# heyblackC/DFMIR

Hardware: AMD Instinct MI355X
Metric: train-step image-pairs/sec (fwd+bwd): 2D 256x256 bs=16 and 3D 160^3 bs=1 (higher is better)
Workload: dtype f32 (fp16x2-split MFMA, fp32 accumulate)

## Files before the change

### dfmir_amd/csrc/conv3x3s.hip

```cpp
#include "split_f16.h"

#ifndef PP_COMPUTE_PRIO
#define PP_COMPUTE_PRIO 1
#endif
#ifndef CS_COMPUTE_PRIO
#define CS_COMPUTE_PRIO 1
#endif
#ifndef CS_STORE_PRIO
#define CS_STORE_PRIO 0
#endif
typedef __bf16 bf16x8 __attribute__((ext_vector_type(8)));
typedef __bf16 bf16x2 __attribute__((ext_vector_type(2)));
typedef _Float16 f16x2 __attribute__((ext_vector_type(2)));
typedef float f32x2 __attribute__((ext_vector_type(2)));

__device__ __forceinline__ unsigned pk_bf16(float a, float b) {
  const f32x2 v = {a, b};
  return __builtin_bit_cast(unsigned, __builtin_convertvector(v, bf16x2));
}

template <int NSP>
__device__ __forceinline__ void split_pair(float x0, float x1, unsigned (&p)[NSP]) {
  if constexpr (NSP == 3) {
    p[0] = pk_bf16(x0, x1);
// ... 581 lines not shown
  const int th = g->Cout > 64 ? 8 : 16;
  const int tx = (g->Wo + CS_TW - 1) / CS_TW, ty = (g->Ho + th - 1) / th;
  const double fill = (double)g->Ho * g->Wo / ((double)tx * CS_TW * ty * th);
  if (!((long long)g->N * tx * ty < (1LL << 31) && fill >= 0.85)) return false;
  *th_out = th; *tx_out = tx; *ty_out = ty;
  return true;
}
static bool split_fwd_geom_ok(const DfConvGeom* g) {
  if (!(g->KD == 1 && g->KH == 3 && g->KW == 3 && g->Di == 1 && g->Do == 1 && g->stride == 1 && g->dil == 1))
    return false;
  if (g->Cout <= 32 || g->Cin < 16 || g->ph != g->pw || g->pd != 0) return false;
  const int p = g->ph;
  if (!(p == 1 || (p == 2 && g->pad_mode == 0))) return false;
  if (g->Ho != g->Hi + 2 * p - 2 || g->Wo != g->Wi + 2 * p - 2) return false;
  const long long HWo = (long long)g->Ho * g->Wo;
  if (HWo >= (1LL << 30) || (long long)g->Hi * g->Wi >= (1LL << 30)) return false;
  if ((long long)((g->Cin + 7) / 8) * 27 * g->Cout * 16 >= (1LL << 31)) return false;
  if (worst_npos(g->Wo, (int)HWo, 128) > 399) return false;
  return true;
}
int df_conv3x3_split_res_ok(const DfConvGeom* g) {
  int th, tx, ty;
  return (df_split_mode() == 2 && split_fwd_geom_ok(g) && cs_plan(g, &th, &tx, &ty)) ? 1 : 0;
}
struct CsLaunch {
  ConvCsP kc;
  dim3 grid;
  int form;
};
static bool cs_setup(const DfConvGeom* g, const float* res, const float* ring, int ring_rl, const float* y, CsLaunch* L) {
  int th = 0, tlx = 0, tly = 0;
  if (!cs_plan(g, &th, &tlx, &tly)) return false;
  ConvCsP kc{g->N, g->Cin, g->Cout, g->Hi, g->Wi, g->Ho, g->Wo, g->ph, g->pad_mode, g->act, g->slope, tlx, tly, res,
             ring, ring_rl, 0, 0, 0};
  kc.vec4 = (g->Wo % 4 == 0 && ((uintptr_t)y & 15) == 0 && ((uintptr_t)res & 15) == 0) ? 1 : 0;
  static DfOptInt dephase_o{"DFMIR_CS_DEPHASE", 0};
  const long long nb = (long long)g->N * tlx * tly;
  if (nb * ((g->Cout + 127) / 128) >= 512) kc.dephase = dephase_o.get();
  static DfOptInt xcd_o{"DFMIR_CS_XCD_PAIR", 2};
  const int xcd_pair = xcd_o.get();
  if (g->Cout > 64) {
    dim3 grid((unsigned)nb, (unsigned)((g->Cout + 127) / 128));
    if (xcd_pair && grid.y <= 2 && (nb & 7) == 0) {
      kc.xcd_pair = xcd_pair == 1 ? (grid.y == 2 ? 1 : 0) : (int)grid.y + 1;
      if (kc.xcd_pair) grid = dim3((unsigned)(grid.y * nb), 1u);
    }
    L->grid = grid;
    L->form = 1;
  } else {
    if (xcd_pair >= 2 && (nb & 7) == 0) kc.xcd_pair = 2;
    L->grid = dim3((unsigned)nb, 1u);
    L->form = 2;
  }
  L->kc = kc;
  return true;
}
bool df_conv3x3_split_fwd_try(const DfConvGeom* g, const float* x, const float* x_amax, int x_n, const float* w_packed,
                              const float* bias, const float* res, const float* ring, int ring_rl, float* y,
                              hipStream_t st, int* rc) {
  const int mode = df_split_mode();
  if (mode == 0 || (mode == 2 && !(x_amax && x_n > 0))) return false;
  if (!split_fwd_geom_ok(g)) return false;
  const int p = g->ph;
  const long long HWo = (long long)g->Ho * g->Wo;
  Conv3P k{g->N, g->Cin, g->Cout, g->Hi, g->Wi, g->Ho, g->Wo, p, g->pad_mode, g->act, g->slope, 0};
  const u32x4* ws = reinterpret_cast<const u32x4*>(split_section(w_packed, g->Cin, g->Cout));
  const SplitScale sc{x_amax, x_n, split_trailer(w_packed, g->Cin, g->Cout, mode)};
  CsLaunch cl;
  if (mode == 2 && cs_setup(g, res, ring, ring_rl, y, &cl)) {
    const ConvCsP& kc = cl.kc;
    if (cl.form == 1) {
#ifdef DFMIR_BUILD_W1
      static DfOptFlag w1_o{"DFMIR_CONV_W1"};
      if (w1_o.get() && kc.vec4 && g->act != 2 && (g->Cin % 16) == 0 && (g->Ho % 16) == 0 && (g->Wo % 32) == 0) {
        ConvCsP kw = kc;
        kw.tiles_y = g->Ho / 16;
        const long long nbw = (long long)g->N * kw.tiles_x * kw.tiles_y;
        const unsigned gyw = (unsigned)((g->Cout + 127) / 128);
        kw.xcd_pair = 0;
        dim3 gw((unsigned)nbw, gyw);
        if ((nbw & 7) == 0 && gyw <= 2) { kw.xcd_pair = (int)gyw + 1; gw = dim3((unsigned)(gyw * nbw), 1u); }
        conv3x3_split_w1_k<0><<<gw, 256, 0, st>>>(x, ws, bias, y, kw, sc);
      } else
#endif
      conv3x3_split_cs_k<64, 8><<<cl.grid, 512, 0, st>>>(x, ws, bias, y, kc, sc);
    } else {
      conv3x3_split_cs_k<32, 16><<<cl.grid, 512, 0, st>>>(x, ws, bias, y, kc, sc);
    }
    hipError_t e = hipGetLastError();
    *rc = (e == hipSuccess) ? 0 : df_set_error((int)e, __FILE__, __LINE__);
    return true;
  }
  if (res || ring) { *rc = df_set_error((int)hipErrorInvalidValue, __FILE__, __LINE__); return true; }
  k.tiles_per_img = (int)((HWo + 255) / 256);
  const bool big = g->Cout > 64;
  dim3 grid((unsigned)(g->N * k.tiles_per_img), big ? (unsigned)((g->Cout + 127) / 128) : 1u);
  if (mode == 2) {
    if (big) conv3x3_split_pp_k<2, 400, 128><<<grid, 512, 0, st>>>(x, ws, bias, y, k, sc);
    else conv3x3_split_pp_k<2, 400, 64><<<grid, 512, 0, st>>>(x, ws, bias, y, k, sc);
  } else {
    if (big) conv3x3_split_pp_k<3, 400, 128><<<grid, 512, 0, st>>>(x, ws, bias, y, k, sc);
    else conv3x3_split_pp_k<3, 400, 64><<<grid, 512, 0, st>>>(x, ws, bias, y, k, sc);
  }
  hipError_t e = hipGetLastError();
  *rc = (e == hipSuccess) ? 0 : df_set_error((int)e, __FILE__, __LINE__);
  return true;
}

struct WS3P {
  int N, Cin, Cout, H, W, pad_mode;
  int runs_per_row, runs_per_img, runs_total, runs_per_block;
  const float* x_amax;
  const float* dy_amax;
  int x_n, dy_n;
  float* db;
  const float* dy_pmax;
  int swap;
  float* dbx;
  const float* fx;
};

template <int NSP, int BC>
__global__ __launch_bounds__(512, 1) void conv3x3_wgrad_split_k(const float* __restrict__ x,
                                                                const float* __restrict__ dy,
                                                                float* __restrict__ dwt, WS3P k) {
  using P = Prod<NSP>;
  constexpr int CT = 64, NWC = BC / 32, KS = 4 / NWC, NSTEP = 18 / KS;
  constexpr int XSLAB = 2 * CT;
  __shared__ __attribute__((aligned(16))) u32x4 Xc[NSP * 3 * 4 * XSLAB];
  __shared__ __attribute__((aligned(16))) u32x4 Dy[NSP * 2 * 2 * BC];
  __shared__ float bsum[BC];

  const int tid = threadIdx.x, lane = tid & 63, wid = tid >> 6;
  const bool want_db = k.db != nullptr && blockIdx.y == 0;
  if (tid < BC) bsum[tid] = 0.f;
  float bacc = 0.f;
  const int wc = wid % NWC, wi = (wid / NWC) & 1, kh = wid / (2 * NWC);
  const int l31 = lane & 31, lhi = lane >> 5;
  const int HW = k.H * k.W;
  const int ci0 = blockIdx.y * CT, co0 = blockIdx.z * BC;
  const int run_beg = blockIdx.x * k.runs_per_block;
  int run_end = run_beg + k.runs_per_block;
  if (run_end > k.runs_total) run_end = k.runs_total;

  float xscale = 1.f, dscale = 1.f, oscale = 1.f, oscale2 = 1.f;
  if (NSP == 2) {
    __shared__ float red[17];
    const int ex = scale_exp(reduce_absmax(k.x_amax, k.x_n, red));
    __syncthreads();
    const int ed = scale_exp(reduce_absmax(k.dy_amax, k.dy_n, red));
    xscale = pow2f(ex); dscale = pow2f(ed); oscale = pow2f(-ex); oscale2 = pow2f(-ed);
  }

  const int xc = tid & 63, xu = (tid >> 6) & 1, xr = tid >> 7;
  const int dc = tid % BC, du = (tid / BC) & 1, dk = (tid / (2 * BC)) & 1;
  const bool dload = tid < 4 * BC;
  const unsigned hw4 = (unsigned)HW * 4u;
  constexpr unsigned OOB = 0x80000000u;

  f32x16 acc[9];
#pragma unroll
  for (int t = 0; t < 9; ++t)
#pragma unroll
    for (int r = 0; r < 16; ++r) acc[t][r] = 0.f;

  u32x4 rxa, rxb, rda, rdb;
  unsigned rxl, rxr;

#define WS_GLOAD(run_)                                                                           \
  {                                                                                              \
    const int n_ = (run_) / k.runs_per_img;                                                      \
    const int q_ = (run_) - n_ * k.runs_per_img;                                                 \
    const int yp_ = q_ / k.runs_per_row, xs_ = q_ - yp_ * k.runs_per_row;                        \
    const int y0_ = 2 * yp_, x0_ = 16 * xs_ + 8 * xu;                                            \
    const __amdgpu_buffer_rsrc_t bx_ = __builtin_amdgcn_make_buffer_rsrc(                        \
        const_cast<float*>(x + (long long)n_ * k.Cin * HW), 0, (unsigned)(k.Cin * HW) * 4u, 0x00020000); \
    const __amdgpu_buffer_rsrc_t bd_ = __builtin_amdgcn_make_buffer_rsrc(                        \
        const_cast<float*>(dy + (long long)n_ * k.Cout * HW), 0, (unsigned)(k.Cout * HW) * 4u, 0x00020000); \
    const bool cok_ = ci0 + xc < k.Cin;                                                          \
    const unsigned cb_ = (unsigned)(ci0 + xc) * hw4;                                             \
     \
                                             \
    int ry_ = y0_ - 1 + xr;                                                                      \
    bool rok_ = (unsigned)ry_ < (unsigned)k.H;                                                   \
    if (k.pad_mode == 1) { ry_ = ry_ < 0 ? -ry_ : (ry_ >= k.H ? 2 * (k.H - 1) - ry_ : ry_); rok_ = true; } \
    const int rb_ = ry_ * k.W;                                                                   \
    const bool lin_ = x0_ > 0, rin_ = x0_ + 8 < k.W;                                             \
    const int ol_ = rb_ + (lin_ ? x0_ - 1 : 1), or_ = rb_ + (rin_ ? x0_ + 8 : k.W - 2);          \
    const bool lok_ = rok_ && cok_ && (lin_ || k.pad_mode == 1), rrok_ = rok_ && cok_ && (rin_ || k.pad_mode == 1); \
    const unsigned xb_ = (rok_ && cok_) ? cb_ + (unsigned)(rb_ + x0_) * 4u : OOB;                \
    rxa = __builtin_amdgcn_raw_buffer_load_b128(bx_, xb_, 0, 0);                                 \
    rxb = __builtin_amdgcn_raw_buffer_load_b128(bx_, xb_ == OOB ? OOB : xb_ + 16u, 0, 0);        \
    rxl = __builtin_amdgcn_raw_buffer_load_b32(bx_, lok_ ? cb_ + (unsigned)ol_ * 4u : OOB, 0, 0); \
    rxr = __builtin_amdgcn_raw_buffer_load_b32(bx_, rrok_ ? cb_ + (unsigned)or_ * 4u : OOB, 0, 0); \
    const unsigned db_ = (co0 + dc >= k.Cout || !dload) ? OOB                                    \
        : (unsigned)(co0 + dc) * hw4 + (unsigned)((y0_ + dk) * k.W + 16 * xs_ + 8 * du) * 4u;    \
    rda = __builtin_amdgcn_raw_buffer_load_b128(bd_, db_, 0, 0);                                 \
    rdb = __builtin_amdgcn_raw_buffer_load_b128(bd_, db_ == OOB ? OOB : db_ + 16u, 0, 0);        \
  }
#define WS_LSTORE()                                                                              \
  {                                                                                              \
    float r[10];                                                                                 \
    r[0] = __uint_as_float(rxl); r[9] = __uint_as_float(rxr);                                    \
    _Pragma("unroll") for (int e = 0; e < 4; ++e) { r[1 + e] = __uint_as_float(rxa[e]); r[5 + e] = __uint_as_float(rxb[e]); } \
    unsigned pa[5][NSP], pb[4][NSP];                                                             \
    _Pragma("unroll") for (int i = 0; i < 5; ++i) split_pair_s<NSP>(r[2 * i], r[2 * i + 1], xscale, pa[i]); \
    if (NSP == 2) {             \
      _Pragma("unroll") for (int i = 0; i < 4; ++i)                                              \
        _Pragma("unroll") for (int s = 0; s < NSP; ++s) pb[i][s] = __builtin_amdgcn_alignbit(pa[i + 1][s], pa[i][s], 16); \
    } else {                                                                                     \
      _Pragma("unroll") for (int i = 0; i < 4; ++i) split_pair<NSP>(r[2 * i + 1], r[2 * i + 2], pb[i]); \
    }                                                                                            \
    _Pragma("unroll") for (int s = 0; s < NSP; ++s) {                                            \
      u32x4* dst = Xc + ((s * 3 * 4 + xr) * 2 + xu) * CT + xc;                                   \
      dst[0] = u32x4{pa[0][s], pa[1][s], pa[2][s], pa[3][s]};                                    \
      dst[4 * XSLAB] = u32x4{pb[0][s], pb[1][s], pb[2][s], pb[3][s]};                            \
      dst[8 * XSLAB] = u32x4{pa[1][s], pa[2][s], pa[3][s], pa[4][s]};                            \
    }                                                                                            \
    float v[8];                                                                                  \
    _Pragma("unroll") for (int e = 0; e < 4; ++e) { v[e] = __uint_as_float(rda[e]); v[4 + e] = __uint_as_float(rdb[e]); } \
    bacc += ((v[0] + v[1]) + (v[2] + v[3])) + ((v[4] + v[5]) + (v[6] + v[7]));    \
    u32x4 sp[NSP];                                                                               \
    split8_s<NSP>(v, dscale, sp);                                                                \
    if (dload) { _Pragma("unroll") for (int s = 0; s < NSP; ++s) Dy[((s * 2 + dk) * 2 + du) * BC + dc] = sp[s]; } \
  }

  if (run_beg < run_end) {
    WS_GLOAD(run_beg);
    WS_LSTORE();
  }
  __syncthreads();

  const int abase = lhi * CT + wi * 32 + l31 + (KS == 2 ? kh * XSLAB : 0);
  const int bbase = lhi * BC + wc * 32 + l31 + (KS == 2 ? kh * 2 * BC : 0);
  for (int run = run_beg; run < run_end; ++run) {
    const bool more = (run + 1) < run_end;
    if (more) WS_GLOAD(run + 1);
    u32x4 b[NSP], a[2][NSP];
#define WS_LOADA(set_, step_)                                                                    \
  _Pragma("unroll") for (int s = 0; s < NSP; ++s)                                                \
    a[set_][s] = Xc[((s * 3 + ((step_) % 3)) * 4 + (step_) / 9 + ((step_) % 9) / 3) * XSLAB + abase];
    WS_LOADA(0, 0)
#pragma unroll
    for (int step = 0; step < NSTEP; ++step) {
      if (step % 9 == 0) {
#pragma unroll
        for (int s = 0; s < NSP; ++s) b[s] = Dy[(s * 2 + step / 9) * 2 * BC + bbase];
      }
      if (step + 1 < NSTEP) WS_LOADA((step + 1) & 1, step + 1)
#pragma unroll
      for (int q = 0; q < P::N; ++q)
        acc[step % 9] = mma16<NSP>(a[step & 1][P::A[q]], b[P::B[q]], acc[step % 9]);
    }
#undef WS_LOADA
#pragma unroll
    for (int i = 0; i < 2 * NSP; ++i) __builtin_amdgcn_sched_group_barrier(0x100, 1, 0);
#pragma unroll
    for (int step = 0; step < NSTEP; ++step) {
      const int nr = (step + 1 < NSTEP ? NSP : 0) + ((step + 1) % 9 == 0 && step + 1 < NSTEP ? NSP : 0);
#pragma unroll
      for (int i = 0; i < P::N; ++i) {
        __builtin_amdgcn_sched_group_barrier(0x008, 1, 0);
        if (i < nr) __builtin_amdgcn_sched_group_barrier(0x100, 1, 0);
        if (i == P::N - 1) {
#pragma unroll
          for (int e = P::N; e < nr; ++e) __builtin_amdgcn_sched_group_barrier(0x100, 1, 0);
        }
      }
    }
    if (more) {
      __syncthreads();
      WS_LSTORE();
      __syncthreads();
    }
  }
#undef WS_GLOAD
#undef WS_LSTORE

  if (want_db) {
    if (dload) atomicAdd(&bsum[dc], bacc);
    __syncthreads();
    if (tid < BC && co0 + tid < k.Cout) atomicAdd(&k.db[co0 + tid], bsum[tid]);
  }
  const int co = co0 + wc * 32 + l31;
  if (co < k.Cout) {
#pragma unroll
    for (int t = 0; t < 9; ++t) {
#pragma unroll
      for (int r = 0; r < 16; ++r) {
        const int ci = ci0 + wi * 32 + 4 * lhi + (r & 3) + 8 * (r >> 2);
        if (ci < k.Cin)
          df_acc(dwt, ((long long)t * k.Cin + ci) * k.Cout + co, NSP == 2 ? acc[t][r] * oscale * oscale2 : acc[t][r], k.fx);
      }
    }
  }
}

struct RingP {
  int N, K, M, H, W;
  int RL;
  const float* cols;
};
constexpr int RING_KG = 32;

template <int RP>
__global__ __launch_bounds__(512) void conv3x3_reflect_ring_k(const float* __restrict__ dy, const u32x4* __restrict__ ws,
                                                              float* __restrict__ ring, RingP k, SplitScale sc) {
  constexpr int NSP = 2;
  using P = Prod<2>;
  __shared__ __attribute__((aligned(16))) u32x4 Ls[NSP * RING_KG * RP];
  __shared__ float red[17];
  const int tid = threadIdx.x, lane = tid & 63;
  const int wid = __builtin_amdgcn_readfirstlane((int)(threadIdx.x >> 6));
  const int l31 = lane & 31, lhi = lane >> 5;
  const int strip = blockIdx.x & 3, n = blockIdx.x >> 2;
  const int m0 = blockIdx.y * 128;
  const bool rowstrip = strip < 2;
  const int L = rowstrip ? k.W : k.H;
  const int HW = k.H * k.W;
  const float* dyl = dy + (long long)n * k.K * HW +
                     (strip == 0 ? 0 : strip == 1 ? (k.H - 1) * k.W : strip == 2 ? 0 : k.W - 1);
  const int istr = rowstrip ? 1 : k.W;

  const int ex = scale_exp(reduce_absmax(sc.x_amax, sc.x_n, red));
  const int ew = (int)sc.w_trailer[1];
  const float xscale = pow2f(ex), oscale = pow2f(-ex), oscale2 = pow2f(-ew);

  const int kg_n = (k.K + 7) >> 3;
  {
    const int npad = RP - L;
    for (int it = tid; it < NSP * RING_KG * npad; it += 512) {
      const int q = it % npad, g = it / npad;
      Ls[g * RP + (q < 2 ? q : L + q)] = u32x4{0u, 0u, 0u, 0u};
    }
    const int kz = RING_KG - kg_n;
    for (int it = tid; it < NSP * kz * L; it += 512) {
      const int i = it % L, g = it / L, s2 = g / kz, kg = kg_n + g % kz;
      Ls[(s2 * RING_KG + kg) * RP + i + 2] = u32x4{0u, 0u, 0u, 0u};
    }
  }
  for (int it = tid; it < kg_n * L; it += 512) {
    const int i = it % L, kg = it / L;
    float v[8];
#pragma unroll
    for (int e = 0; e < 8; ++e) {
      const int kk = kg * 8 + e;
      if (!rowstrip && k.cols) v[e] = kk < k.K ? k.cols[(((long long)n * k.K + kk) * 2 + (strip - 2)) * k.H + i] : 0.f;
      else v[e] = kk < k.K ? dyl[(long long)kk * HW + (long long)i * istr] : 0.f;
    }
    u32x4 sp[NSP];
    split8_s<NSP>(v, xscale, sp);
#pragma unroll
    for (int s = 0; s < NSP; ++s) Ls[(s * RING_KG + kg) * RP + i + 2] = sp[s];
  }
  __syncthreads();

  const int mb = wid & 3, kh = wid >> 2;
  const int m = m0 + mb * 32 + l31;
  const int nb_n = (L + 2 + 31) >> 5;
  f32x16 acc[3];
#pragma unroll
  for (int b = 0; b < 3; ++b)
#pragma unroll
    for (int r = 0; r < 16; ++r) acc[b][r] = 0.f;
  const int chunks = (k.K + 15) >> 4;
  const int tap0 = strip == 0 ? 6 : strip == 1 ? 0 : strip == 2 ? 2 : 0, tapd = rowstrip ? 1 : 3;
  u32x4 a[3][NSP], an[3][NSP], an2[3][NSP];
#define RING_LOADA(dst_, c_)                                                                     \
  {                                                                                              \
    const int kg_ = 2 * (c_) + lhi;                                                              \
    const bool ok_ = (c_) < chunks && kg_ < kg_n && m < k.M;                                     \
    _Pragma("unroll") for (int j = 0; j < 3; ++j)                                                \
      _Pragma("unroll") for (int s = 0; s < NSP; ++s)                                            \
        dst_[j][s] = ok_ ? ws[((long long)kg_ * NSP * 9 + s * 9 + tap0 + j * tapd) * k.M + m] : u32x4{0u, 0u, 0u, 0u}; \
  }
  RING_LOADA(a, kh)
  RING_LOADA(an, kh + 2)
  for (int c = kh; c < chunks; c += 2) {
    RING_LOADA(an2, c + 4)
    const int kg = 2 * c + lhi;
#pragma unroll
    for (int j = 0; j < 3; ++j) {
#pragma unroll
      for (int b = 0; b < 3; ++b) {
        if (b < nb_n) {
          int pos = b * 32 + l31 + j;
          pos = pos < RP ? pos : RP - 1;
          u32x4 x2[NSP];
#pragma unroll
          for (int s = 0; s < NSP; ++s) x2[s] = Ls[(s * RING_KG + kg) * RP + pos];
#pragma unroll
          for (int q = 0; q < P::N; ++q) acc[b] = mma16<NSP>(a[j][P::A[q]], x2[P::B[q]], acc[b]);
        }
      }
    }
#pragma unroll
    for (int j = 0; j < 3; ++j)
#pragma unroll
      for (int s = 0; s < NSP; ++s) { a[j][s] = an[j][s]; an[j][s] = an2[j][s]; }
  }
#undef RING_LOADA

  __syncthreads();
  float* xch = reinterpret_cast<float*>(Ls);
  if (kh == 1) {
#pragma unroll
    for (int b = 0; b < 3; ++b)
#pragma unroll
      for (int r = 0; r < 16; ++r) xch[((mb * 3 + b) * 16 + r) * 64 + lane] = acc[b][r];
  }
  __syncthreads();
  if (kh == 1) return;
  float* rg = ring + ((long long)(n * 4 + strip) * k.M) * k.RL;
#pragma unroll
  for (int b = 0; b < 3; ++b) {
    if (b >= nb_n) continue;
    const int c = b * 32 + l31;
    if (c > L + 1) continue;
#pragma unroll
    for (int r = 0; r < 16; ++r) {
      const int mm = m0 + mb * 32 + 4 * lhi + (r & 3) + 8 * (r >> 2);
      if (mm < k.M)
        rg[(long long)mm * k.RL + c] = (acc[b][r] + xch[((mb * 3 + b) * 16 + r) * 64 + lane]) * oscale * oscale2;
    }
  }
}

int df_conv3x3_reflect_ring_ok(const DfConvGeom* g) {
  if (df_split_mode() != 2) return 0;
  if (!(g->KD == 1 && g->KH == 3 && g->KW == 3 && g->Di == 1 && g->Do == 1 && g->stride == 1 && g->dil == 1)) return 0;
  if (g->pad_mode != 1 || g->ph != 1 || g->pw != 1 || g->pd != 0) return 0;
  if (g->Ho != g->Hi || g->Wo != g->Wi || g->Hi < 4 || g->Wi < 4 || g->Hi > 94 || g->Wi > 94) return 0;
  if (g->Cout > 8 * RING_KG || g->Cout < 16 || g->Cin <= 32) return 0;
  return 1;
}
int df_conv3x3_reflect_ring_len(const DfConvGeom* g) { return ((g->Hi > g->Wi ? g->Hi : g->Wi) + 2 + 3) & ~3; }
int df_conv3x3_reflect_ring_launch(const DfConvGeom* g, const float* dy, const float* dy_cols, const float* dy_amax,
                                   int dy_n, const float* wd_packed, float* ring, hipStream_t st) {
  const RingP k{g->N, g->Cout, g->Cin, g->Hi, g->Wi, df_conv3x3_reflect_ring_len(g), dy_cols};
  const u32x4* ws = reinterpret_cast<const u32x4*>(split_section(wd_packed, g->Cout, g->Cin));
  const SplitScale sc{dy_amax, dy_n, split_trailer(wd_packed, g->Cout, g->Cin, 2)};
  const dim3 grid((unsigned)(4 * g->N), (unsigned)((g->Cin + 127) / 128));
  if (g->Hi <= 64 && g->Wi <= 64) conv3x3_reflect_ring_k<72><<<grid, 512, 0, st>>>(dy, ws, ring, k, sc);
  else conv3x3_reflect_ring_k<100><<<grid, 512, 0, st>>>(dy, ws, ring, k, sc);
  return (int)hipGetLastError();
}

#ifdef W2_TRACE
__device__ unsigned g_w2_trace[8 * 64 * 8];
extern "C" int dfmir_w2_trace_dump(unsigned* out) {
  return (int)hipMemcpyFromSymbol(out, HIP_SYMBOL(g_w2_trace), sizeof(g_w2_trace));
}
#define W2T(slot_) { if (trace_blk && lane == 0 && run - run_beg < 64) g_w2_trace[(wid * 64 + (run - run_beg)) * 8 + (slot_)] = (unsigned)__builtin_readcyclecounter(); }
#define W2T_VM() { __builtin_amdgcn_s_waitcnt(0x0f70); W2T(4) }
#else
#define W2T(slot_)
#define W2T_VM()
#endif
#ifndef W2_ALT
#define W2_ALT 0
#endif
#ifndef W2_PRIO_C
#define W2_PRIO_C 0
#endif
#ifndef W2_PRIO_G0
#define W2_PRIO_G0 1
#endif
#ifndef W2_PRIO_G1
#define W2_PRIO_G1 2
#endif
#ifndef W2_CTPAD
#define W2_CTPAD 0
#endif
struct W2Lds {
  static constexpr int XCU = 2 * 3 * 4 * 2 * (64 + W2_CTPAD), DYU = 2 * 2 * 2 * 128;
  static constexpr int DY_OFF = 2 * XCU * 16, EDC_OFF = DY_OFF + 2 * DYU * 16, RED_OFF = EDC_OFF + 128 * 4, BYTES = RED_OFF + 80;
};
__global__ __launch_bounds__(512, 1) void conv3x3_wgrad_split2_k(const float* __restrict__ x,
                                                                 const float* __restrict__ dy,
                                                                 float* __restrict__ dwt, WS3P k) {
  __shared__ __attribute__((aligned(16))) u32x4 Xc[2 * W2Lds::XCU];
  __shared__ __attribute__((aligned(16))) u32x4 Dy[2 * W2Lds::DYU];
  __shared__ float red[17];
  __shared__ int edc[128];
  const unsigned bix = blockIdx.x, biy = blockIdx.y, biz = blockIdx.z;
#include "conv3x3s_w2_body.inc"
}

bool df_conv3x3_split_wgrad_swaps(const DfConvGeom* g) {
  return df_split_mode() == 2 && g->KD == 1 && g->KH == 3 && g->KW == 3 && g->Di == 1 && g->Do == 1 && g->stride == 1 &&
         g->dil == 1 && g->ph == 1 && g->pw == 1 && g->pd == 0 && g->Ho == g->Hi && g->Wo == g->Wi && g->pad_mode == 0 &&
         g->Cout == 64 && g->Cin > 64;
}
static bool ws_setup(const DfConvGeom* g, const float* x_amax, int x_n, const float* dy_amax, int dy_n, float* db,
                     const float* dy_pmax, WS3P* kp, dim3* grid, int* which) {
  const int mode = df_split_mode();
  if (mode == 0 || (mode == 2 && !(x_amax && dy_amax && x_n > 0 && dy_n > 0))) return false;
  if (!(g->KD == 1 && g->KH == 3 && g->KW == 3 && g->Di == 1 && g->Do == 1 && g->stride == 1 && g->dil == 1))
    return false;
  if (g->ph != 1 || g->pw != 1 || g->pd != 0 || g->Ho != g->Hi || g->Wo != g->Wi) return false;
  if (g->Cout < 64 || g->Cin < 64) return false;
  const bool wide = g->Cout > 64;
  if ((g->Hi & 1) || (g->Wi & 15) || g->Hi < 2) return false;
  const long long HW = (long long)g->Hi * g->Wi;
  if (HW * g->Cin * 4 >= (1LL << 31) || HW * g->Cout * 4 >= (1LL << 31)) return false;
  const bool swap = mode == 2 && x_amax && dy_amax && df_conv3x3_split_wgrad_swaps(g);
  WS3P k{g->N, g->Cin, g->Cout, g->Hi, g->Wi, g->pad_mode, g->Wi / 16, 0, 0, 0, x_amax, dy_amax, x_n, dy_n, db, dy_pmax, 0, nullptr, df_det_fx()};
  if (swap) {
    k.Cin = g->Cout; k.Cout = g->Cin;
    k.x_amax = dy_amax; k.dy_amax = x_amax; k.x_n = dy_n; k.dy_n = x_n;
    k.db = nullptr; k.dbx = db; k.dy_pmax = nullptr; k.swap = 1;
  }
  k.runs_per_img = (g->Hi / 2) * k.runs_per_row;
  const long long total = (long long)g->N * k.runs_per_img;
  if (total >= (1LL << 30)) return false;
  k.runs_total = (int)total;
  const unsigned ny = (k.Cin + 63) / 64, nz = (wide || swap) ? (k.Cout + 127) / 128 : 1;
  long long want = 256 / ((long long)ny * nz);
  if (want < 1) want = 1;
  long long maxs = (k.runs_total + 7) / 8;
  if (maxs < 1) maxs = 1;
  if (want > maxs) want = maxs;
  k.runs_per_block = (int)((k.runs_total + want - 1) / want);
  const unsigned nx = (k.runs_total + k.runs_per_block - 1) / k.runs_per_block;
  *grid = dim3(nx, ny, nz);
  *kp = k;
  if (mode == 2) *which = swap ? 1 : wide ? 2 : 3;
  else *which = wide ? 4 : 5;
  return true;
}
bool df_conv3x3_split_wgrad_try(const DfConvGeom* g, const float* x, const float* x_amax, int x_n, const float* dy,
                                const float* dy_amax, int dy_n, float* dw_tcc, float* db, hipStream_t st, int* rc,
                                const float* dy_pmax) {
  WS3P k;
  dim3 grid;
  int which = 0;
  if (!ws_setup(g, x_amax, x_n, dy_amax, dy_n, db, dy_pmax, &k, &grid, &which)) return false;
  if (which == 1) conv3x3_wgrad_split2_k<<<grid, 512, 0, st>>>(dy, x, dw_tcc, k);
  else if (which == 2) conv3x3_wgrad_split2_k<<<grid, 512, 0, st>>>(x, dy, dw_tcc, k);
  else if (which == 3) conv3x3_wgrad_split_k<2, 64><<<grid, 512, 0, st>>>(x, dy, dw_tcc, k);
  else if (which == 4) conv3x3_wgrad_split_k<3, 128><<<grid, 512, 0, st>>>(x, dy, dw_tcc, k);
  else conv3x3_wgrad_split_k<3, 64><<<grid, 512, 0, st>>>(x, dy, dw_tcc, k);
  hipError_t e = hipGetLastError();
  *rc = (e == hipSuccess) ? 0 : df_set_error((int)e, __FILE__, __LINE__);
  return true;
}

struct PairP {
  int order;
  int nd, ndx;
  int nw, nwx, nwy;
  int gd, gw;
};
template <int CPG, int TH>
__global__ __launch_bounds__(512, 1) void conv3x3_bwd_pair_k(const float* __restrict__ dyd, const u32x4* __restrict__ ws,
                                                             float* __restrict__ dx, ConvCsP kc, SplitScale sc,
                                                             const float* __restrict__ xw, const float* __restrict__ dyw,
                                                             float* __restrict__ dwt, WS3P kw, PairP pp) {
  constexpr int LDS_B = CsLds<CPG, TH>::BYTES > W2Lds::BYTES ? CsLds<CPG, TH>::BYTES : W2Lds::BYTES;
  __shared__ __attribute__((aligned(16))) unsigned char lds[LDS_B];
  const int id = (int)blockIdx.x;
  bool wg;
  int l;
  if (pp.order == 0) {
    wg = id < 8 * pp.gw;
    l = wg ? id : id - 8 * pp.gw;
  } else if (pp.order == 1) {
    wg = id >= 8 * pp.gd;
    l = wg ? id - 8 * pp.gd : id;
  } else {
    const unsigned long long g = (unsigned)id >> 3, tot = (unsigned)(pp.gd + pp.gw);
    const int wb = (int)(g * (unsigned)pp.gw / tot);
    wg = (int)((g + 1) * (unsigned)pp.gw / tot) > wb;
    l = ((wg ? wb : (int)g - wb) << 3) | (id & 7);
  }
  if (!wg) {
    if (l >= pp.nd) return;
    using L = CsLds<CPG, TH>;
    const float* __restrict__ x = dyd;
    const float* __restrict__ bias = nullptr;
    float* __restrict__ y = dx;
    const ConvCsP& k = kc;
    const int bix = l % pp.ndx, biy = l / pp.ndx, gdx = pp.ndx;
    u32x4 (*Wg)[L::WUG] = reinterpret_cast<u32x4 (*)[L::WUG]>(lds);
    u32x4 (*Xs)[L::XSU] = reinterpret_cast<u32x4 (*)[L::XSU]>(lds + L::XS_OFF);
    float* bs = reinterpret_cast<float*>(lds + L::BS_OFF);
#include "conv3x3s_cs_body.inc"
  } else {
    if (l >= pp.nw) return;
    const float* __restrict__ x = xw;
    const float* __restrict__ dy = dyw;
    const WS3P& k = kw;
    const int t = l / pp.nwx;
    const unsigned bix = (unsigned)(l - t * pp.nwx), biy = (unsigned)(t % pp.nwy), biz = (unsigned)(t / pp.nwy);
    u32x4* Xc = reinterpret_cast<u32x4*>(lds);
    u32x4* Dy = reinterpret_cast<u32x4*>(lds + W2Lds::DY_OFF);
    int* edc = reinterpret_cast<int*>(lds + W2Lds::EDC_OFF);
    float* red = reinterpret_cast<float*>(lds + W2Lds::RED_OFF);
#include "conv3x3s_w2_body.inc"
  }
}

#ifndef DF_BWD_PAIR_DEFAULT
#define DF_BWD_PAIR_DEFAULT 1
#endif
#ifndef DF_BWD_PAIR_ORDER_DEFAULT
#define DF_BWD_PAIR_ORDER_DEFAULT 1
#endif
static bool bwd_pair_enabled() {
  static DfOptFlag no_o{"DFMIR_NO_BWD_PAIR"};
  static DfOptInt on_o{"DFMIR_BWD_PAIR", DF_BWD_PAIR_DEFAULT};
  return !no_o.get() && on_o.get() != 0;
}
static bool bwd_pair_setup(const DfConvGeom* gd, const DfConvGeom* gw, const float* dy_amax, int dy_n, const float* x_amax,
                           int x_n, const float* res, const float* ring, int ring_rl, const float* dx, float* db,
                           const float* dy_pmax, CsLaunch* cl, WS3P* kw, dim3* wgrid, int* which) {
  if (!bwd_pair_enabled() || df_split_mode() != 2) return false;
  if (!(gd->N == gw->N && gd->Cin == gw->Cout && gd->Cout == gw->Cin && gd->Hi == gw->Ho && gd->Wi == gw->Wo &&
        gd->Ho == gw->Hi && gd->Wo == gw->Wi && gd->act == 0))
    return false;
  if (!(dy_amax && dy_n > 0 && x_amax && x_n > 0)) return false;
#ifdef DFMIR_BUILD_W1
  static DfOptFlag w1_o{"DFMIR_CONV_W1"};
  if (w1_o.get()) return false;
#endif
  if (!split_fwd_geom_ok(gd) || !cs_setup(gd, res, ring, ring_rl, dx, cl)) return false;
  if (!ws_setup(gw, x_amax, x_n, dy_amax, dy_n, db, dy_pmax, kw, wgrid, which) || *which > 2 || kw->fx != nullptr) return false;
  const long long nd = (long long)cl->grid.x * cl->grid.y, nw = (long long)wgrid->x * wgrid->y * wgrid->z;
  return nd + nw + 16 < (1LL << 31);
}
int df_conv3x3_bwd_pair_ok(const DfConvGeom* gd, const DfConvGeom* gw) {
  static const float one = 1.f;
  CsLaunch cl;
  WS3P kw;
  dim3 wgrid;
  int which = 0;
  return bwd_pair_setup(gd, gw, &one, 1, &one, 1, nullptr, nullptr, 0, nullptr, nullptr, nullptr, &cl, &kw, &wgrid, &which) ? 1 : 0;
}
bool df_conv3x3_bwd_pair_try(const DfConvGeom* gd, const DfConvGeom* gw, const float* dy, const float* dy_amax, int dy_n,
                             const float* dy_pmax, const float* wd_packed, const float* res, const float* ring, int ring_rl,
                             float* dx, const float* x, const float* x_amax, int x_n, float* dw_tcc, float* db,
                             hipStream_t st, int* rc) {
  CsLaunch cl;
  WS3P kw;
  dim3 wgrid;
  int which = 0;
  if (!bwd_pair_setup(gd, gw, dy_amax, dy_n, x_amax, x_n, res, ring, ring_rl, dx, db, dy_pmax, &cl, &kw, &wgrid, &which))
    return false;
  static DfOptInt order_o{"DFMIR_BWD_PAIR_ORDER", DF_BWD_PAIR_ORDER_DEFAULT};
  int order = order_o.get();
  if (order < 0 || order > 2) order = DF_BWD_PAIR_ORDER_DEFAULT;
  const u32x4* ws = reinterpret_cast<const u32x4*>(split_section(wd_packed, gd->Cin, gd->Cout));
  const SplitScale sc{dy_amax, dy_n, split_trailer(wd_packed, gd->Cin, gd->Cout, 2)};
  PairP pp;
  pp.order = order;
  pp.nd = (int)(cl.grid.x * cl.grid.y); pp.ndx = (int)cl.grid.x;
  pp.nw = (int)(wgrid.x * wgrid.y * wgrid.z); pp.nwx = (int)wgrid.x; pp.nwy = (int)wgrid.y;
  pp.gd = (pp.nd + 7) >> 3; pp.gw = (pp.nw + 7) >> 3;
  const dim3 grid((unsigned)(8 * (pp.gd + pp.gw)));
  const float* xw = which == 1 ? dy : x;
  const float* dyw = which == 1 ? x : dy;
  if (cl.form == 1) conv3x3_bwd_pair_k<64, 8><<<grid, 512, 0, st>>>(dy, ws, dx, cl.kc, sc, xw, dyw, dw_tcc, kw, pp);
  else conv3x3_bwd_pair_k<32, 16><<<grid, 512, 0, st>>>(dy, ws, dx, cl.kc, sc, xw, dyw, dw_tcc, kw, pp);
  hipError_t e = hipGetLastError();
  *rc = (e == hipSuccess) ? 0 : df_set_error((int)e, __FILE__, __LINE__);
  return true;
}
```

Before: 215.7.

## Add ring2 reflect-conv kernel with early global loads, deeper weight prefetch, split epilogue

Adds a second ring kernel for the 3x3 reflect-padding boundary strips, which becomes the default path. It issues the strip's global loads into registers before the amax reduction so their latency overlaps the scale computation. Weights are prefetched PF chunks ahead, with PF chosen from the block count relative to the CU count. The cross-wave reduction in the epilogue is also split so both K-halves store half the rows instead of one wave idling. The cost is more registers (launch bounds set occupancy per PF) and extra template variants; the old kernel stays reachable behind an env flag, and timing-trace hooks are added under a macro.

```diff
diff --git a/dfmir_amd/csrc/conv3x3s.hip b/dfmir_amd/csrc/conv3x3s.hip
--- a/dfmir_amd/csrc/conv3x3s.hip
+++ b/dfmir_amd/csrc/conv3x3s.hip
@@ -907,6 +907,17 @@
   const float* cols;
 };
 constexpr int RING_KG = 32;
+#ifdef RING_TRACE
+__device__ unsigned long long g_ring_trace[256 * 8];
+__device__ unsigned g_ring_trace_n;
+extern "C" int dfmir_ring_trace_dump(unsigned long long* out, unsigned* n) {
+  const int rc = (int)hipMemcpyFromSymbol(out, HIP_SYMBOL(g_ring_trace), sizeof(g_ring_trace));
+  return rc ? rc : (int)hipMemcpyFromSymbol(n, HIP_SYMBOL(g_ring_trace_n), sizeof(unsigned));
+}
+#define RING_T(slot_) { if (rt) { __builtin_amdgcn_sched_barrier(0); rt[slot_] = __builtin_amdgcn_s_memrealtime(); __builtin_amdgcn_sched_barrier(0); } }
+#else
+#define RING_T(slot_)
+#endif
 
 template <int RP>
 __global__ __launch_bounds__(512) void conv3x3_reflect_ring_k(const float* __restrict__ dy, const u32x4* __restrict__ ws,
@@ -926,8 +937,20 @@
   const float* dyl = dy + (long long)n * k.K * HW +
                      (strip == 0 ? 0 : strip == 1 ? (k.H - 1) * k.W : strip == 2 ? 0 : k.W - 1);
   const int istr = rowstrip ? 1 : k.W;
+#ifdef RING_TRACE
+  unsigned long long* rt = nullptr;
+  if (tid == 0 && blockIdx.x == gridDim.x / 2 && blockIdx.y == 0) {
+    const unsigned slot = atomicAdd(&g_ring_trace_n, 1u);
+    if (slot < 256) {
+      rt = g_ring_trace + slot * 8;
+      rt[5] = k.N; rt[6] = ((unsigned long long)k.K << 16) | k.M; rt[7] = ((unsigned long long)k.H << 16) | k.W;
+    }
+  }
+#endif
+  RING_T(0)
 
   const int ex = scale_exp(reduce_absmax(sc.x_amax, sc.x_n, red));
+  RING_T(1)
   const int ew = (int)sc.w_trailer[1];
   const float xscale = pow2f(ex), oscale = pow2f(-ex), oscale2 = pow2f(-ew);
 
@@ -959,6 +982,7 @@
     for (int s = 0; s < NSP; ++s) Ls[(s * RING_KG + kg) * RP + i + 2] = sp[s];
   }
   __syncthreads();
+  RING_T(2)
 
   const int mb = wid & 3, kh = wid >> 2;
   const int m = m0 + mb * 32 + l31;
@@ -1005,6 +1029,7 @@
       for (int s = 0; s < NSP; ++s) { a[j][s] = an[j][s]; an[j][s] = an2[j][s]; }
   }
 #undef RING_LOADA
+  RING_T(3)
 
   __syncthreads();
   float* xch = reinterpret_cast<float*>(Ls);
@@ -1029,6 +1054,199 @@
         rg[(long long)mm * k.RL + c] = (acc[b][r] + xch[((mb * 3 + b) * 16 + r) * 64 + lane]) * oscale * oscale2;
     }
   }
+#ifdef RING_TRACE
+  asm volatile("s_waitcnt vmcnt(0)" ::: "memory");
+#endif
+  RING_T(4)
+}
+
+template <int RP, int PF>
+__global__ __launch_bounds__(512, PF == 1 ? 4 : 2) void conv3x3_reflect_ring2_k(const float* __restrict__ dy,
+                                                                                 const u32x4* __restrict__ ws,
+                                                                                 float* __restrict__ ring, RingP k, SplitScale sc) {
+  constexpr int NSP = 2;
+  using P = Prod<2>;
+  constexpr int LMAX = RP == 72 ? 64 : 94;
+  constexpr int NIT = (RING_KG * LMAX + 511) / 512;
+  __shared__ __attribute__((aligned(16))) u32x4 Ls[NSP * RING_KG * RP];
+  const int tid = threadIdx.x, lane = tid & 63;
+  const int wid = __builtin_amdgcn_readfirstlane((int)(threadIdx.x >> 6));
+  const int l31 = lane & 31, lhi = lane >> 5;
+  const int strip = blockIdx.x & 3, n = blockIdx.x >> 2;
+  const int m0 = blockIdx.y * 128;
+  const bool rowstrip = strip < 2;
+  const int L = rowstrip ? k.W : k.H;
+  const int HW = k.H * k.W;
+  const int kg_n = (k.K + 7) >> 3;
+  const bool from_cols = !rowstrip && k.cols != nullptr;
+  const float* lp = from_cols ? k.cols + ((long long)n * k.K * 2 + (strip - 2)) * k.H
+                              : dy + (long long)n * k.K * HW +
+                                    (strip == 0 ? 0 : strip == 1 ? (k.H - 1) * k.W : strip == 2 ? 0 : k.W - 1);
+  const long long lsk = from_cols ? 2 * k.H : HW;
+  const int lsi = (rowstrip || from_cols) ? 1 : k.W;
+#ifdef RING_TRACE
+  unsigned long long* rt = nullptr;
+  if (tid == 0 && blockIdx.x == gridDim.x / 2 && blockIdx.y == 0) {
+    const unsigned slot = atomicAdd(&g_ring_trace_n, 1u);
+    if (slot < 256) {
+      rt = g_ring_trace + slot * 8;
+      rt[5] = k.N; rt[6] = ((unsigned long long)k.K << 16) | k.M; rt[7] = ((unsigned long long)k.H << 16) | k.W;
+    }
+  }
+#endif
+  RING_T(0)
+
+  float lv[NIT][8];
+#pragma unroll
+  for (int t = 0; t < NIT; ++t) {
+    const int it = tid + t * 512;
+    const int i = it % L, kg = it / L;
+#pragma unroll
+    for (int e = 0; e < 8; ++e) {
+      int kk = kg * 8 + e;
+      kk = kk < k.K ? kk : k.K - 1;
+      lv[t][e] = lp[(long long)kk * lsk + (long long)i * lsi];
+    }
+  }
+  float am;
+  if (sc.x_n <= 1) am = sc.x_amax[0];
+  else {
+    am = 0.f;
+    for (int i = lane; i < sc.x_n; i += 64) am = fmaxf(am, sc.x_amax[i]);
+#pragma unroll
+    for (int o = 32; o > 0; o >>= 1) am = fmaxf(am, __shfl_xor(am, o, 64));
+  }
+  const int ex = scale_exp(am);
+  RING_T(1)
+  const int ew = (int)sc.w_trailer[1];
+  const float xscale = pow2f(ex), oscale = pow2f(-ex), oscale2 = pow2f(-ew);
+
+  {
+    const int npad = RP - L;
+    for (int it = tid; it < NSP * RING_KG * npad; it += 512) {
+      const int q = it % npad, g = it / npad;
+      Ls[g * RP + (q < 2 ? q : L + q)] = u32x4{0u, 0u, 0u, 0u};
+    }
+    const int kz = RING_KG - kg_n;
+    for (int it = tid; it < NSP * kz * L; it += 512) {
+      const int i = it % L, g = it / L, s2 = g / kz, kg = kg_n + g % kz;
+      Ls[(s2 * RING_KG + kg) * RP + i + 2] = u32x4{0u, 0u, 0u, 0u};
+    }
+  }
+
+  const int mb = wid & 3, kh = wid >> 2;
+  const int m = m0 + mb * 32 + l31;
+  const int mc = m < k.M ? m : k.M - 1;
+  const int chunks = (k.K + 15) >> 4;
+  const int tap0 = strip == 0 ? 6 : strip == 1 ? 0 : strip == 2 ? 2 : 0, tapd = rowstrip ? 1 : 3;
+  u32x4 wq[PF + 1][3][NSP];
+#define RING_LOADA(dst_, c_)                                                                     \
+  {                                                                                              \
+    const int kg_ = 2 * (c_) + lhi;                                                              \
+    const bool ok_ = (c_) < chunks && kg_ < kg_n && m < k.M;                                     \
+    const int kgc_ = kg_ < kg_n ? kg_ : kg_n - 1;                                                \
+    _Pragma("unroll") for (int j = 0; j < 3; ++j)                                                \
+      _Pragma("unroll") for (int s = 0; s < NSP; ++s) {                                          \
+        const u32x4 t_ = ws[((long long)kgc_ * NSP * 9 + s * 9 + tap0 + j * tapd) * k.M + mc];   \
+        dst_[j][s] = ok_ ? t_ : u32x4{0u, 0u, 0u, 0u};                                           \
+      }                                                                                          \
+  }
+#pragma unroll
+  for (int f = 0; f < PF; ++f) RING_LOADA(wq[f], kh + 2 * f)
+
+#pragma unroll
+  for (int t = 0; t < NIT; ++t) {
+    const int it = tid + t * 512;
+    const int i = it % L, kg = it / L;
+    if (it < kg_n * L) {
+      float v[8];
+#pragma unroll
+      for (int e = 0; e < 8; ++e) v[e] = kg * 8 + e < k.K ? lv[t][e] : 0.f;
+      u32x4 sp[NSP];
+      split8_s<NSP>(v, xscale, sp);
+#pragma unroll
+      for (int s = 0; s < NSP; ++s) Ls[(s * RING_KG + kg) * RP + i + 2] = sp[s];
+    }
+  }
+  __syncthreads();
+  RING_T(2)
+
+  const int nb_n = (L + 2 + 31) >> 5;
+  f32x16 acc[3];
+#pragma unroll
+  for (int b = 0; b < 3; ++b)
+#pragma unroll
+    for (int r = 0; r < 16; ++r) acc[b][r] = 0.f;
+#if defined(RING_TRACE) && RING_TRACE == 3
+  u32x4 xko[NSP];
+#pragma unroll
+  for (int s = 0; s < NSP; ++s) xko[s] = Ls[(s * RING_KG + lhi) * RP + l31];
+#endif
+  for (int c = kh; c < chunks; c += 2) {
+#if !(defined(RING_TRACE) && RING_TRACE == 2)
+    RING_LOADA(wq[PF], c + 2 * PF)
+#endif
+    const int kg = 2 * c + lhi;
+#pragma unroll
+    for (int j = 0; j < 3; ++j) {
+#pragma unroll
+      for (int b = 0; b < 3; ++b) {
+        if (b < nb_n) {
+          int pos = b * 32 + l31 + j;
+          pos = pos < RP ? pos : RP - 1;
+          u32x4 x2[NSP];
+#if defined(RING_TRACE) && RING_TRACE == 3
+#pragma unroll
+          for (int s = 0; s < NSP; ++s) { x2[s] = xko[s]; x2[s][0] += (unsigned)(pos + kg); }
+#else
+#pragma unroll
+          for (int s = 0; s < NSP; ++s) x2[s] = Ls[(s * RING_KG + kg) * RP + pos];
+#endif
+#pragma unroll
+          for (int q = 0; q < P::N; ++q) acc[b] = mma16<NSP>(wq[0][j][P::A[q]], x2[P::B[q]], acc[b]);
+        }
+      }
+    }
+#if !(defined(RING_TRACE) && RING_TRACE == 2)
+#pragma unroll
+    for (int f = 0; f < PF; ++f)
+#pragma unroll
+      for (int j = 0; j < 3; ++j)
+#pragma unroll
+        for (int s = 0; s < NSP; ++s) wq[f][j][s] = wq[f + 1][j][s];
+#endif
+  }
+#undef RING_LOADA
+  RING_T(3)
+
+  __syncthreads();
+  float* xch = reinterpret_cast<float*>(Ls);
+#pragma unroll
+  for (int b = 0; b < 3; ++b)
+#pragma unroll
+    for (int r = 0; r < 16; ++r)
+      if ((r >> 3) != kh) xch[((mb * 3 + b) * 16 + r) * 64 + lane] = acc[b][r];
+  __syncthreads();
+  float* rg = ring + ((long long)(n * 4 + strip) * k.M) * k.RL;
+#pragma unroll
+  for (int b = 0; b < 3; ++b) {
+    if (b >= nb_n) continue;
+    const int c = b * 32 + l31;
+    if (c > L + 1) continue;
+#pragma unroll
+    for (int r = 0; r < 16; ++r) {
+      if ((r >> 3) != kh) continue;
+      const int mm = m0 + mb * 32 + 4 * lhi + (r & 3) + 8 * (r >> 2);
+      if (mm < k.M) {
+        const float mine = acc[b][r], other = xch[((mb * 3 + b) * 16 + r) * 64 + lane];
+        rg[(long long)mm * k.RL + c] = ((kh == 0 ? mine + other : other + mine)) * oscale * oscale2;
+      }
+    }
+  }
+#ifdef RING_TRACE
+  asm volatile("s_waitcnt vmcnt(0)" ::: "memory");
+#endif
+  RING_T(4)
 }
 
 int df_conv3x3_reflect_ring_ok(const DfConvGeom* g) {
@@ -1046,8 +1264,17 @@
   const u32x4* ws = reinterpret_cast<const u32x4*>(split_section(wd_packed, g->Cout, g->Cin));
   const SplitScale sc{dy_amax, dy_n, split_trailer(wd_packed, g->Cout, g->Cin, 2)};
   const dim3 grid((unsigned)(4 * g->N), (unsigned)((g->Cin + 127) / 128));
-  if (g->Hi <= 64 && g->Wi <= 64) conv3x3_reflect_ring_k<72><<<grid, 512, 0, st>>>(dy, ws, ring, k, sc);
-  else conv3x3_reflect_ring_k<100><<<grid, 512, 0, st>>>(dy, ws, ring, k, sc);
+  static DfOptFlag v1_o{"DFMIR_RING_V1"};
+  if (v1_o.get()) {
+    if (g->Hi <= 64 && g->Wi <= 64) conv3x3_reflect_ring_k<72><<<grid, 512, 0, st>>>(dy, ws, ring, k, sc);
+    else conv3x3_reflect_ring_k<100><<<grid, 512, 0, st>>>(dy, ws, ring, k, sc);
+  } else if (!(g->Hi <= 64 && g->Wi <= 64)) {
+    conv3x3_reflect_ring2_k<100, 3><<<grid, 512, 0, st>>>(dy, ws, ring, k, sc);
+  } else if ((long long)grid.x * grid.y > df_cu_count()) {
+    conv3x3_reflect_ring2_k<72, 1><<<grid, 512, 0, st>>>(dy, ws, ring, k, sc);
+  } else {
+    conv3x3_reflect_ring2_k<72, 3><<<grid, 512, 0, st>>>(dy, ws, ring, k, sc);
+  }
   return (int)hipGetLastError();
 }
 
```

After: 216.8, median of 6. Within noise of the previous version (+0.5%).
